# tombultreys/ptv_interpolation

Measured on AMD Instinct MI355X. Metric: Mvoxels/s interpolated + achieved HBM GB/s, 512³ grid / 5M particles IDW, higher is better.
Workload: dtype f64

## Files before the change

### include/ptv_api.h

```cpp
#ifndef PTV_API_H
#define PTV_API_H

#include <stdint.h>

#ifdef __cplusplus
extern "C" {
#endif

#define PTV_API_VERSION 11

#define PTV_OK 0
#define PTV_E_ARG -1
#define PTV_E_HIP -2
#define PTV_E_NOMEM -3
#define PTV_E_UNSUPPORTED -4
#define PTV_E_INEXACT -5
#define PTV_E_SINGULAR -6

#define PTV_METHOD_IDW 0
#define PTV_METHOD_SIBSON 1
#define PTV_METHOD_NEAREST 2
#define PTV_METHOD_IDW_RADIUS 3

#define PTV_RBF_LINEAR 0
// ... 238 lines not shown
typedef struct {
    int64_t n_fluid, n_dirichlet;
    int32_t itn;
    int32_t info;
    int32_t solver;
    int32_t anchor_plane;
    double bnorm, rnorm;
    double sum_abs_fx, sum_abs_fy, sum_abs_fz, sum_w;
    double ms_force, ms_divergence, ms_solve;
    double ms_iter_median;
    double ms_total;
} ptv_pressure_stats;

int ptv_version(void);
int ptv_abi_sizes(int64_t out6[6]);
int ptv_abi_sizes2(int64_t out3[3]);
int ptv_abi_sizes3(int64_t out1[1]);
int ptv_abi_sizes4(int64_t out2[2]);
int ptv_abi_sizes5(int64_t out2[2]);
int ptv_abi_sizes6(int64_t out2[2]);
int ptv_abi_sizes7(int64_t out2[2]);
int ptv_abi_sizes8(int64_t out4[4]);
int ptv_abi_sizes9(int64_t out2[2]);
const char *ptv_last_error(void);
int ptv_device_count(int *out);
int ptv_init(int device, ptv_ctx **out);
int ptv_free(ptv_ctx *ctx);

int ptv_interp_knn(ptv_ctx *ctx, const ptv_particles *p, const ptv_grid *g,
                   const ptv_knn_params *prm, double *U, double *V, double *W,
                   ptv_stats *st);

int ptv_interp_knn_dev(ptv_ctx *ctx, const ptv_particles *p, const ptv_grid *g,
                       const ptv_knn_params *prm, double *U, double *V, double *W,
                       void *stream, ptv_stats *st);

int ptv_interp_rbf_local(ptv_ctx *ctx, const ptv_particles *p, const ptv_grid *g,
                         const ptv_rbf_params *prm, double *U, double *V, double *W,
                         ptv_stats *st);

int ptv_interp_rbf_local_dev(ptv_ctx *ctx, const ptv_particles *p, const ptv_grid *g,
                             const ptv_rbf_params *prm, double *U, double *V, double *W,
                             void *stream, ptv_stats *st);

int ptv_interp_linear(ptv_ctx *ctx, const ptv_particles *p, const ptv_grid *g,
                      const ptv_linear_params *prm, double *U, double *V, double *W,
// ... 97 lines not shown
                         const double *Fz, double *D);

int ptv_force_divergence_dev(ptv_ctx *ctx, const ptv_pressure_params *prm, const double *Fx, const double *Fy,
                             const double *Fz, double *D, void *stream);

int ptv_poisson_solve(ptv_ctx *ctx, const ptv_pressure_params *prm, const double *rhs, const double *Fx,
                      const double *Fy, const double *Fz, const uint8_t *dirichlet, double *X,
                      ptv_pressure_stats *st);

int ptv_poisson_solve_dev(ptv_ctx *ctx, const ptv_pressure_params *prm, const double *rhs, const double *Fx,
                          const double *Fy, const double *Fz, const uint8_t *dirichlet, double *X, void *stream,
                          ptv_pressure_stats *st);

int ptv_pressure_recover(ptv_ctx *ctx, const ptv_pressure_params *prm, const double *U, const double *V,
                         const double *W, double *P, ptv_pressure_stats *st);

int ptv_pressure_recover_dev(ptv_ctx *ctx, const ptv_pressure_params *prm, const double *U, const double *V,
                             const double *W, double *P, void *stream, ptv_pressure_stats *st);

int ptv_last_stats(ptv_ctx *ctx, ptv_stats *st);

int ptv_debug_stamps(ptv_ctx *ctx, int mode, double *out23);

#ifdef __cplusplus
}
#endif

#endif
```

### ptv_interpolation_amd/_lib.py

```python
from __future__ import annotations

import ctypes as C
import os
import threading

import numpy as np

HERE = os.path.dirname(os.path.abspath(__file__))
_DEFAULT_LIB = os.path.join(HERE, "libptv_amd.so")
LIB_PATH = os.environ.get("PTV_LIB", _DEFAULT_LIB)

PTV_OK = 0
PTV_E_ARG = -1
PTV_E_HIP = -2
PTV_E_NOMEM = -3
PTV_E_UNSUPPORTED = -4
PTV_E_INEXACT = -5
PTV_E_SINGULAR = -6

METHOD_IDW = 0
METHOD_SIBSON = 1
METHOD_NEAREST = 2
METHOD_IDW_RADIUS = 3

# ... 282 lines not shown
    "ptv_interface_drag": (C.c_int, [C.c_void_p, C.POINTER(DragParams)] + [C.c_void_p] * 6 + [_dp]),
    "ptv_interface_drag_dev": (C.c_int, [C.c_void_p, C.POINTER(DragParams)] + [C.c_void_p] * 7 + [_dp]),
    "ptv_gradient_sums": (C.c_int, [C.c_void_p, C.POINTER(FlowParams), C.c_void_p, _dp]),
    "ptv_gradient_sums_dev": (C.c_int, [C.c_void_p, C.POINTER(FlowParams), C.c_void_p, C.c_void_p, _dp]),
    "ptv_abi_sizes8": (C.c_int, [C.POINTER(C.c_int64)]),
    "ptv_edt": (C.c_int, [C.c_void_p, C.POINTER(EdtParams)] + [C.c_void_p] * 3 + [C.POINTER(EdtStats)]),
    "ptv_edt_dev": (C.c_int, [C.c_void_p, C.POINTER(EdtParams)] + [C.c_void_p] * 4 + [C.POINTER(EdtStats)]),
    "ptv_align_score": (C.c_int, [C.c_void_p, C.POINTER(AlignParams)] + [C.c_void_p] * 4 + [_dp]),
    "ptv_align_score_dev": (C.c_int, [C.c_void_p, C.POINTER(AlignParams)] + [C.c_void_p] * 5 + [_dp]),
    "ptv_abi_sizes9": (C.c_int, [C.POINTER(C.c_int64)]),
    "ptv_force_field": (C.c_int, [C.c_void_p, C.POINTER(PressureParams)] + [_dp] * 6 + [C.POINTER(PressureStats)]),
    "ptv_force_field_dev": (C.c_int, [C.c_void_p, C.POINTER(PressureParams)] + [_dp] * 6 +
                            [C.c_void_p, C.POINTER(PressureStats)]),
    "ptv_force_divergence": (C.c_int, [C.c_void_p, C.POINTER(PressureParams)] + [_dp] * 4),
    "ptv_force_divergence_dev": (C.c_int, [C.c_void_p, C.POINTER(PressureParams)] + [_dp] * 4 + [C.c_void_p]),
    "ptv_poisson_solve": (C.c_int, [C.c_void_p, C.POINTER(PressureParams)] + [_dp] * 4 + [_u8p, _dp,
                                                                                           C.POINTER(PressureStats)]),
    "ptv_poisson_solve_dev": (C.c_int, [C.c_void_p, C.POINTER(PressureParams)] + [_dp] * 4 +
                              [_u8p, _dp, C.c_void_p, C.POINTER(PressureStats)]),
    "ptv_pressure_recover": (C.c_int, [C.c_void_p, C.POINTER(PressureParams)] + [_dp] * 4 +
                             [C.POINTER(PressureStats)]),
    "ptv_pressure_recover_dev": (C.c_int, [C.c_void_p, C.POINTER(PressureParams)] + [_dp] * 4 +
                                 [C.c_void_p, C.POINTER(PressureStats)]),
    "ptv_last_stats": (C.c_int, [C.c_void_p, C.POINTER(Stats)]),
    "ptv_debug_stamps": (C.c_int, [C.c_void_p, C.c_int, C.POINTER(C.c_double)]),
}

_lib = None
_lock = threading.Lock()


class PtvError(RuntimeError):
    def __init__(self, code, msg):
        super().__init__(f"ptv error {code}: {msg}")
        self.code = code
        self.msg = msg


def lib():
    global _lib
    with _lock:
        if _lib is None:
            if not os.path.exists(LIB_PATH):
                raise ImportError(
                    f"{LIB_PATH} not found: build it with `python -m ptv_interpolation_amd.build` "
                    "(hipcc, gfx950). The k-NN path has no CPU fallback.")
# ... 74 lines not shown
    out = (C.c_int64 * 2)()
    check(lib().ptv_abi_sizes6(out))
    return list(out), [C.sizeof(FlowParams), C.sizeof(FlowStats)]


def abi_sizes7():
    out = (C.c_int64 * 2)()
    check(lib().ptv_abi_sizes7(out))
    return list(out), [C.sizeof(DragParams), C.sizeof(DragStats)]


def abi_sizes8():
    out = (C.c_int64 * 4)()
    check(lib().ptv_abi_sizes8(out))
    return list(out), [C.sizeof(EdtParams), C.sizeof(EdtStats), C.sizeof(AlignParams), C.sizeof(AlignRecord)]


def abi_sizes9():
    out = (C.c_int64 * 2)()
    check(lib().ptv_abi_sizes9(out))
    return list(out), [C.sizeof(PressureParams), C.sizeof(PressureStats)]


def edt_check_shape(shape):
    if len(shape) != 3:
        raise NotImplementedError(f"the GPU distance transform is 3-D only (got {len(shape)}-D)")
    if sum(int(n) * int(n) for n in shape) >= 2**31:
        raise NotImplementedError(f"shape {tuple(shape)}: nz^2 + ny^2 + nx^2 must be below 2^31 "
                                  "(squared distances are 32-bit on the GPU)")
    return tuple(int(n) for n in shape)


def drag_label_table(labels):
    lab = np.asarray(labels)
    if lab.ndim != 1 or lab.size == 0:
        raise ValueError("labels must be a non-empty 1-D sequence")
    if lab.dtype.kind not in "biu":
        raise NotImplementedError(f"labels of dtype {lab.dtype} (GPU path: integers or bool)")
    lab = lab.astype(np.int64) if lab.dtype != np.uint64 else lab
    if lab.max() > np.iinfo(np.int32).max or lab.min() < np.iinfo(np.int32).min:
        raise NotImplementedError("labels outside the int32 range are not supported on the GPU path")
    if lab.min() <= 0:
        raise NotImplementedError("labels must be positive on the GPU path (0 is the fluid)")
    table, slot = np.unique(lab.astype(np.int32), return_inverse=True)
    return np.ascontiguousarray(table), slot.reshape(-1)

# ... 107 lines not shown
        check(L.ptv_init(int(device), C.byref(h)))
        self.h = h
        self.device = int(device)

    @classmethod
    def get(cls, device: int = 0) -> "Context":
        with _lock:
            ctx = cls._cache.get(device)
        if ctx is None:
            ctx = cls(device)
            with _lock:
                cls._cache[device] = ctx
        return ctx

    def close(self):
        if self.h:
            lib().ptv_free(self.h)
            self.h = None

    def last_stats(self) -> dict:
        st = Stats()
        check(lib().ptv_last_stats(self.h, C.byref(st)))
        return st.as_dict()

    def debug_stamps(self, mode=2):
        out = (C.c_double * 23)()
        check(lib().ptv_debug_stamps(self.h, int(mode), out))
        keys = ("setup", "seeds", "rows", "copy", "compute", "epilogue", "candidates", "merges", "rounds",
                "passes", "kept")
        v = list(out)
        return {"waves": v[0], "mean": dict(zip(keys, v[1:12])), "max": dict(zip(keys, v[12:23]))}

    def sample_mask(self, raw, raw_axes, axes=None, grid_points=None, shape=None, z_range=None):
        rw = np.ascontiguousarray(raw, dtype=np.uint8)
        rnz, rny, rnx = rw.shape
        rax, ray, raz = (np.ascontiguousarray(a, dtype=np.float64).ravel() for a in raw_axes)
        M = MaskGrid(rnx, rny, rnz, rw.ctypes.data_as(_u8p), as_dp(rax), as_dp(ray), as_dp(raz))
        keep = [rw, rax, ray, raz]
        if axes is not None:
            ax, ay, az = (np.ascontiguousarray(a, dtype=np.float64).ravel() for a in axes)
            nx, ny, nz = len(ax), len(ay), len(az)
            keep += [ax, ay, az]
            G = Grid(nx, ny, nz, as_dp(ax), as_dp(ay), as_dp(az), None, None, None, 0, nz)
        else:
            nz, ny, nx = shape
            gp = [np.ascontiguousarray(a, dtype=np.float64).ravel() for a in grid_points]
# ... 626 lines not shown
```

### ptv_interpolation_amd/build.py

```python
from __future__ import annotations

import os
import shutil
import subprocess
import sys
from concurrent.futures import ThreadPoolExecutor

HERE = os.path.dirname(os.path.abspath(__file__))
CSRC = os.path.join(HERE, "csrc")
INCLUDE = os.path.join(os.path.dirname(HERE), "include")
LIB = os.path.join(HERE, "libptv_amd.so")
BUILD = os.path.join(HERE, "csrc", "_build")
KNN_PARTS = ["ptv_knn_k" + g + ".hip" for g in "abcdefgh"]
SOURCES = (["ptv_api.cpp", "ptv_search.cpp", "ptv_run_knn.cpp", "ptv_run_chunked.cpp", "ptv_bin.hip", "ptv_knn.hip"] + KNN_PARTS +
           ["ptv_rbf.hip"] + ["ptv_rbf_ns_" + g + ".hip" for g in "abcd"] +
           ["ptv_div.hip", "ptv_flow.hip", "ptv_drag.hip", "ptv_edt.hip", "ptv_clean.hip", "ptv_variational.hip", "ptv_pressure.hip", "ptv_mask.hip", "ptv_filter.hip", "ptv_linear.hip", "ptv_knn_big.hip"])
ARCH = os.environ.get("PTV_OFFLOAD_ARCH", "gfx950")
EXTRA = {f: ["-mllvm", "-pragma-unroll-threshold=1000000"] for f in ["ptv_rbf.hip"] + ["ptv_rbf_ns_" + g + ".hip" for g in "abcd"]}
for _f in ["ptv_rbf.hip"] + ["ptv_rbf_ns_" + g + ".hip" for g in "abcd"]:
    EXTRA[_f] += ["-mllvm", "-disable-machine-licm"]

COMMON = ["-O3", "-fPIC", "-std=c++17", "-ffp-contract=off", f"--offload-arch={ARCH}",
          "-I", INCLUDE, "-I", CSRC, "-Wno-unused-result"]
EXTRA_FLAGS = os.environ.get("PTV_EXTRA_FLAGS", "").split()
TAG = os.environ.get("PTV_BUILD_TAG", "")
if TAG:
    LIB = os.path.join(os.path.dirname(HERE), "ab", f"libptv_{TAG}.so")
    BUILD = os.path.join(HERE, "csrc", "_build_" + TAG)
    EXTRA_FLAGS.append("-DPTV_DEV_KNOBS=1")


def hipcc() -> str:
    for cand in (os.environ.get("HIPCC"), shutil.which("hipcc"), "/opt/rocm/bin/hipcc"):
        if cand and os.path.exists(cand):
            return cand
    raise RuntimeError("hipcc not found (ROCm toolchain required to build libptv_amd.so)")

# ... 44 lines not shown
```

### ptv_interpolation_amd/csrc/ptv_api.cpp

```cpp
#include <cstdio>
#include <hip/hip_runtime.h>

#include <algorithm>
#include <cmath>
#include <memory>
#include <string>
#include <thread>

#include <sys/mman.h>
#include <vector>

#include "ptv_ctx.hpp"

namespace ptv {

static thread_local std::string g_last_error;
void set_error(const std::string &msg) { g_last_error = msg; }

}

using namespace ptv;

extern "C" {

// ... 72 lines not shown
    out2[1] = (int64_t)sizeof(ptv_drag_stats);
    return PTV_OK;
}

int ptv_abi_sizes8(int64_t out4[4]) {
    if (!out4) {
        set_error("ptv_abi_sizes8: out is NULL");
        return PTV_E_ARG;
    }
    out4[0] = (int64_t)sizeof(ptv_edt_params);
    out4[1] = (int64_t)sizeof(ptv_edt_stats);
    out4[2] = (int64_t)sizeof(ptv_align_params);
    out4[3] = (int64_t)sizeof(ptv_align_record);
    return PTV_OK;
}

int ptv_abi_sizes9(int64_t out2[2]) {
    if (!out2) {
        set_error("ptv_abi_sizes9: out is NULL");
        return PTV_E_ARG;
    }
    out2[0] = (int64_t)sizeof(ptv_pressure_params);
    out2[1] = (int64_t)sizeof(ptv_pressure_stats);
    return PTV_OK;
}

const char *ptv_last_error(void) { return g_last_error.c_str(); }

int ptv_device_count(int *out) {
    if (!out) {
        set_error("ptv_device_count: out is NULL");
        return PTV_E_ARG;
    }
    int n = 0;
    hipError_t e = hipGetDeviceCount(&n);
    if (e != hipSuccess) n = 0;
    *out = n;
    return PTV_OK;
}

int ptv_init(int device, ptv_ctx **out) {
    if (!out) {
        set_error("ptv_init: out is NULL");
        return PTV_E_ARG;
    }
    *out = nullptr;
// ... 501 lines not shown
            if (r[0] == 0 && r[2] == 0 && r[5] == 0) continue;
            ++nrec;
            double v[nv];
            for (int f = 0; f < 6; ++f) v[f] = (double)r[f];
            v[6] = (double)(r[6] & 0xffffffffULL);
            v[7] = (double)(r[6] >> 32);
            v[8] = (double)(r[7] & 0xffffULL);
            v[9] = (double)((r[7] >> 16) & 0xffffULL);
            v[10] = (double)(r[7] >> 32);
            for (int f = 0; f < nv; ++f) {
                sum[f] += v[f];
                mx[f] = std::max(mx[f], v[f]);
            }
        }
        out[0] = (double)nrec;
        for (int f = 0; f < nv; ++f) {
            out[1 + f] = nrec ? sum[f] / (double)nrec : 0.0;
            out[1 + nv + f] = mx[f];
        }
    }
    return PTV_OK;
}

int ptv_divergence_dev(ptv_ctx *c, const ptv_div_params *prm, const void *U, const void *V, const void *W,
                       void *out, void *stream, ptv_stats *st) {
    DivArgs a{};
    PTV_TRY(div_args(c, prm, U, V, W, out, a));
    hipStream_t s = stream ? (hipStream_t)stream : c->stream;
    PTV_TRY(run_div(c, a, U, V, W, prm->fluid_mask, out, s));
    c->last.n_voxels = (prm->z_end - prm->z_begin) * prm->nx * prm->ny;
    if (st) *st = c->last;
    return PTV_OK;
}

int ptv_divergence(ptv_ctx *c, const ptv_div_params *prm, const void *U, const void *V, const void *W, void *out,
                   ptv_stats *st) {
    DivArgs a{};
    PTV_TRY(div_args(c, prm, U, V, W, out, a));
    hipStream_t s = c->stream;
    Event ev[4];
    const size_t ts = a.field_f32 ? 4 : 8, rs = a.result_f32 ? 4 : 8;
    const int64_t nfull = prm->nz * prm->nx * prm->ny;
    const int64_t nout = (prm->z_end - prm->z_begin) * prm->nx * prm->ny;
    PTV_TRY(ev[0].record(s));
    const void *src[3] = {U, V, W};
    for (int i = 0; i < 3; ++i) {
// ... 1352 lines not shown
```

### ptv_interpolation_amd/csrc/ptv_ctx.hpp

```cpp
#pragma once

#include <vector>

#include "../../include/ptv_api.h"
#include "ptv_clean.hpp"
#include "ptv_kernels.hpp"
#include "ptv_knn_big.hpp"
#include "ptv_own.hpp"
#include "ptv_pressure.hpp"
#include "ptv_variational.hpp"

namespace ptv {

constexpr int kMaxLattice = 6;

struct CullCache {
    std::vector<double> key;
    std::vector<double> key_host;
    DevBuf<double> key_dev;
    bool kept_valid = false;
    int64_t kept = 0;
    double bbox[6] = {0, 0, 0, 0, 0, 0};
};

}

struct ptv_ctx {
    int device = 0;
    ptv::Stream stream;
    ptv::Event ev_knn0, ev_knn1, ev_bin0, ev_bin1, ev_lat1;
    ptv::Event ev_main0, ev_cull0, ev_cull1;
    bool cull_timed = false;
    bool timed_pending = false;
    ptv::BigScratch big;
    ptv::DevBuf<double> pin[6], axes, qpts[3], out[3];
    ptv::DevBuf<double> rbf_huge;
    ptv::DevBuf<uint8_t> mask;
    ptv::DevBuf<uint32_t> code, perm, count, start, scanp;
    ptv::DevBuf<uint32_t> bin_keys;
    ptv::DevBuf<uint8_t> bin_temp;
    ptv::DevBuf<double4> prec, pval;
    ptv::DevBuf<double> bbox_part, bbox_out;
    ptv::DevBuf<unsigned long long> dbg;
    ptv::DevBuf<double> lat_axes[ptv::kMaxLattice], lat_dk[ptv::kMaxLattice];
    ptv::DevBuf<float4> lat_recs[ptv::kMaxLattice];
    ptv::DevBuf<int> lat_order[ptv::kMaxLattice];
    ptv::DevBuf<double> lat_okeys;
    ptv::DevBuf<uint32_t> lat_split;
    ptv::DevBuf<double> cmap[2], cdk, ccols, cfp;
    ptv::DevBuf<unsigned long long> ckeys;
    ptv::CullMap cmap_geo{};
    int cdk_n[3] = {0, 0, 0};
    bool cmap_valid = false;
    ptv::CullCache ccache;
    ptv::DevBuf<uint32_t> slots;
    ptv::DevBuf<int> rbf_pw, rbf_status;
    ptv::DevBuf<uint32_t> rbf_nslist;
    ptv::DevBuf<int> rbf_cflag;
    ptv::DevBuf<double> smooth;
    ptv::DevBuf<uint8_t> fld[4];
    ptv::DevBuf<double> mask_axes;
    ptv::DevBuf<int> mask_tabs;
    ptv::DevBuf<uint8_t> mask_raw, mask_out;
    ptv::DevBuf<uint8_t> bnd_ping, bnd_pong;
    ptv::DevBuf<unsigned long long> bnd_counts;
    ptv::DevBuf<double> bnd_xyz;
    ptv::DevBuf<uint8_t> flt_keep;
    ptv::DevBuf<uint32_t> flt_code, flt_perm, flt_count, flt_start, flt_scanp;
    ptv::DevBuf<double> flt_kth, flt_spd;
    ptv::DevBuf<double> cull[6], cull_win;
// ... 119 lines not shown
```

### ptv_interpolation_amd/csrc/ptv_kernels.hpp

```cpp
#pragma once

#include "../../include/ptv_api.h"
#include "ptv_common.hpp"

namespace ptv {

int launch_bbox(const double *const px[3], int64_t n, const double *const qa[3], const int64_t qn[3],
                double *d_partials, int max_blocks, double *d_out6, hipStream_t s,
                const uint32_t *d_n = nullptr);

struct BinSortScratch {
    uint32_t *keys = nullptr;
    void *temp = nullptr;
    size_t temp_bytes = 0;
};
size_t bin_sort_temp_bytes(int64_t n, size_t m);
int launch_bin(const CellGrid &cg, const double *const px[3], const double *const pv[3], int64_t n,
               uint32_t *d_code, uint32_t *d_perm, uint32_t *d_count, uint32_t *d_start,
               uint32_t *d_scan_partials, double4 *d_prec, double4 *d_pval, hipStream_t s,
               const BinSortScratch *ss = nullptr);

size_t scan_partials_needed(size_t m);

size_t cull_blocks(int64_t n);
// ... 51 lines not shown
    int method;
    int k;
    double power, eps;
    uint32_t flags;
    double r0;
    int mode = kModeInterp;
    CoarseBound cb;
    float4 *kd_recs = nullptr;
    int lz0 = -1;
    uint32_t *slots = nullptr;
    double radius = 0.0;
    FilterEpilogue fe;
    const int *order = nullptr;
    unsigned int *rep_cnt = nullptr;
    uint32_t *rep_list = nullptr;
    int rep_cap = 0;
    unsigned int *h_rep = nullptr;
    int64_t *n_repair = nullptr;
    const unsigned long long *gate = nullptr;
    double gate_halo = 0.0;
    int split = 0;
    int split_blocks = 0;
    uint32_t *split_out = nullptr;
};

inline size_t kdist_split_slots(int split, int split_blocks, int kmax) {
    return (size_t)split_blocks * 4 * (size_t)split * (size_t)kmax * 64;
}

int launch_block_order(const double *dk_coarse, const int nc[3], int nx, int ny, int nz, double unit, int *order,
                       double *keys, hipStream_t s);

int launch_count_bound(const CellGrid &g, const uint32_t *cstart, const double *ax, const double *ay,
                       const double *az, int nx, int ny, int nz, int k, double r0, double *out, hipStream_t s);

int launch_subsample(const double *in, int n, int step, double *out, int nout, hipStream_t s);
constexpr int kMaxSubsampleLevels = 8;
struct SubsampleBatch {
    const double *base[3];
    int n0[3];
    int nlev;
    int n[kMaxSubsampleLevels][3];
    double *out[kMaxSubsampleLevels][3];
};
int launch_subsample_levels(const SubsampleBatch &b, int step, hipStream_t s);
int launch_concat3(const double *a, int na, const double *b, int nb, const double *c, int nc, double *out,
                   hipStream_t s);

int launch_halo_need(const double *lax, const double *lay, const double *laz, int nx, int ny, int nz,
                     const double *dk, const double *win, double mg, unsigned long long *out, hipStream_t s);

int kmax_for(int k);
extern unsigned long long *g_dbg;
extern long long g_dbg_cap;

int launch_knn(const KnnLaunch &a, const Binned &b, const double *ax, const double *ay, const double *az,
               const double *qx, const double *qy, const double *qz, const uint8_t *mask, double *U, double *V,
               double *W, hipStream_t s);

struct DivArgs {
    int nx, ny, nz;
    int z_begin, z_end;
    int edge_lo, edge_hi;
    int field_f32;
    int result_f32;
    double dx, dy, dz;
    int ntx = 0, nty = 0, ntiles = 0;
    int xcd = 0;
};

int launch_divergence(const DivArgs &a, const void *U, const void *V, const void *W, const uint8_t *M, void *out,
                      hipStream_t s);

constexpr int kFlowRows = 16;
struct FlowArgs {
    int nx, ny, nz;
    int z_begin, z_end;
// ... 163 lines not shown
```

### ptv_interpolation_amd/csrc/ptv_knn.hip

```cpp
#include "ptv_knn_impl.hpp"

namespace ptv {

unsigned long long *g_dbg = nullptr;
long long g_dbg_cap = 0;

__device__ __forceinline__ int count_inside(const CellGrid &g, const uint32_t *__restrict__ cstart, double qx,
                                            double qy, double qz, double R, int lane) {
    const double Ri = R - g.mg;
    if (Ri <= 0.0) return 0;
    const double R2 = Ri * Ri;
    const int ry0 = clampi(floor((qy - Ri - g.o[1]) * g.ic[1]), g.nc[1]);
    const int ry1 = clampi(floor((qy + Ri - g.o[1]) * g.ic[1]), g.nc[1]);
    const int rz0 = clampi(floor((qz - Ri - g.o[2]) * g.ic[2]), g.nc[2]);
    const int rz1 = clampi(floor((qz + Ri - g.o[2]) * g.ic[2]), g.nc[2]);
    const int nyr = ry1 - ry0 + 1;
    const int nrows = nyr * (rz1 - rz0 + 1);
    int cnt = 0;
    for (int row = lane; row < nrows; row += 64) {
        const int ccy = ry0 + row % nyr, ccz = rz0 + row / nyr;
        const double y0 = g.o[1] + (double)ccy * g.cs[1], y1 = g.o[1] + (double)(ccy + 1) * g.cs[1];
        const double z0 = g.o[2] + (double)ccz * g.cs[2], z1 = g.o[2] + (double)(ccz + 1) * g.cs[2];
        const double fy = fmax(fabs(y0 - qy), fabs(y1 - qy)), fz = fmax(fabs(z0 - qz), fabs(z1 - qz));
        const double h2 = fy * fy + fz * fz;
// ... 343 lines not shown
        diag2 += e * e;
    }
    ka.rall = sqrt(diag2) * (1.0 + 1e-9) + a.cg.mg;
    const long long nblocks = (long long)ka.ntxb * ka.nty * ka.ntz;
    if (nblocks > 0x7fffffffLL || (keys && nblocks >= (1LL << 30))) {
        set_error("grid too large for one launch");
        return PTV_E_ARG;
    }
    ka.nblocks = (int)nblocks;
    int B = 1;
    while (B < 31 && (1LL << B) < b.n) ++B;
    ka.smask = (uint32_t)((1ULL << B) - 1ULL);
    ka.kscale = 1.0 + std::ldexp(1.0, B - 51);
    ka.rep_cnt = nullptr;
    ka.rep_list = nullptr;
    ka.rep_cap = 0;
    ka.tiles = nullptr;
    ka.ntiles = 0;
    ka.split = 0;
    ka.split_tiles = 0;
    ka.split_out = nullptr;
    ka.split_lb = 0;
    ka.order_skip = 0;
    if (a.mode == kModeKDist && a.split > 1 && a.split_blocks > 0 && a.order != nullptr && a.split_out != nullptr) {
        const int nsb = (int)std::min<long long>(a.split_blocks, nblocks);
        KnnKernelArgs ks = ka;
        ks.split = a.split;
        ks.split_tiles = nsb * 4;
        ks.split_out = a.split_out;
        PTV_HIP(hipMemsetAsync(a.split_out, 0xff, kdist_split_slots(a.split, nsb, km) * sizeof(uint32_t), s));
        const long long sblocks = ((long long)ks.split_tiles * a.split + 3) / 4;
        const long long total = sblocks + (nblocks - nsb);
        if (total > 0x7fffffffLL) {
            set_error("split lattice launch too large");
            return PTV_E_ARG;
        }
        ks.nblocks = (int)total;
        ks.split_lb = (int)sblocks;
        ks.order_skip = (int)(nsb - sblocks);
        int rc = launch_kmax(km, false, grid_for(total), s, ks, b, ax, ay, az, qx, qy, qz, mask, U, V, W);
        if (rc != PTV_OK) return rc;
        ks.mode = kModeKDistMerge;
        return launch_kmax(km, false, grid_for(nsb), s, ks, b, ax, ay, az, qx, qy, qz, mask, U, V, W);
    }
    const bool repair = keys && a.mode != kModeKDist && a.mode != kModeRadius;
    if (repair) {
// ... 30 lines not shown
```

### ptv_interpolation_amd/csrc/ptv_knn_impl.hpp

```cpp
#pragma once
#include <hip/hip_runtime.h>

#include <cfloat>
#include <cstdlib>
#include <algorithm>
#include <cmath>
#include <utility>

#include "../../include/ptv_api.h"
#include "ptv_kernels.hpp"
#include "ptv_median.hpp"
#include "ptv_wave.hpp"

namespace ptv {

#ifndef PTV_SUBBALL_RUNS
#define PTV_SUBBALL_RUNS 1
#endif
#ifndef PTV_KNN_WAVES
#define PTV_KNN_WAVES 4
#endif
#ifndef PTV_KNN_WAVES_BIG
#define PTV_KNN_WAVES_BIG 2
#endif
// ... 81 lines not shown
    CoarseBound cb;
    float4 *kd_recs;
    int lz0;
    uint32_t *slots;
    int seed_n;
    int nblocks;
    double radius;
    FilterEpilogue fe;
    const int *order;
    uint32_t smask;
    double kscale;
    unsigned int *rep_cnt;
    uint32_t *rep_list;
    int rep_cap;
    const uint32_t *tiles;
    int ntiles;
    const unsigned long long *gate;
    double gate_halo;
    int split;
    int split_tiles;
    uint32_t *split_out;
    int split_lb;
    int order_skip;
};

__device__ __forceinline__ double make_key(bool has, double e2, uint32_t slot, uint32_t smask) {
    const unsigned long long bits = (unsigned long long)__double_as_longlong(e2);
    uint32_t lo = ((uint32_t)bits & ~smask) | slot;
    uint32_t hi = (uint32_t)(bits >> 32);
    lo = has ? lo : 0u;
    hi = has ? hi : 0x7ff00000u;
    return __longlong_as_double((long long)(((unsigned long long)hi << 32) | lo));
}

__device__ __forceinline__ uint32_t key_slot(double key, uint32_t smask) {
    return (uint32_t)__double_as_longlong(key) & smask;
}

__device__ __forceinline__ bool same_trunc(double a, double b, uint32_t smask) {
    const unsigned long long x = (unsigned long long)(__double_as_longlong(a) ^ __double_as_longlong(b));
    return (x & ~(unsigned long long)smask) == 0ull;
}

template <int KMAX>
__device__ __forceinline__ void insert_key(double (&bd)[KMAX], double key) {
    double cd = key;
// ... 1832 lines not shown
```

### ptv_interpolation_amd/csrc/ptv_search.cpp

```cpp
#include <algorithm>
#include <cmath>
#include <cstdio>
#include <cstdlib>
#include <cstring>
#include <vector>

#include "ptv_ctx.hpp"

namespace ptv {

namespace {

constexpr double kDefaultOccupancySmallK = 16.0;
constexpr double kDefaultXRefSmallK = 12.0;
constexpr double kDefaultOccupancy = 1.2;
constexpr double kDefaultOccupancyLargeK = 8.0;
constexpr double kDefaultXRefLargeK = 4.0;
constexpr double kDefaultR0Scale = 1.0;
constexpr long long kMaxCells = 1LL << 28;
constexpr long long kLatticeStopPoints = 50000;
constexpr size_t kSeedBytesMax = 40ULL << 30;
constexpr int kLatticeSplit = 16;
constexpr long long kLatticeSplitMinBlocks = 64;
constexpr long long kLatticeSplitDiv = 128;
// ... 220 lines not shown
            if (!lattice_level_above(nl) && !(exact_finest && nlat == 1 && nmin >= 2)) break;
            Lat &L = lat[nlat];
            for (int d = 0; d < 3; ++d) L.n[d] = n[d] <= 1 ? 1 : (n[d] - 1 + kLatticeStep - 1) / kLatticeStep + 1;
            PTV_TRY(c->lat_axes[nlat].ensure((size_t)L.n[0] + L.n[1] + L.n[2]));
            PTV_TRY(c->lat_dk[nlat].ensure((size_t)L.n[0] * L.n[1] * L.n[2]));
            L.ax = c->lat_axes[nlat].p;
            L.ay = L.ax + L.n[0];
            L.az = L.ay + L.n[1];
            L.dk = c->lat_dk[nlat].p;
            L.recs = nullptr;
            double *dst[3] = {L.ax, L.ay, L.az};
            for (int d = 0; d < 3; ++d) {
                sb.n[nlat][d] = L.n[d];
                sb.out[nlat][d] = dst[d];
                n[d] = L.n[d];
            }
            ++nlat;
        }
        sb.nlev = nlat;
        if (nlat > 0) PTV_TRY(launch_subsample_levels(sb, kLatticeStep, s));
    }

    const KnnLaunch kl = search_launch(g, prm, pr);
    PTV_TRY(c->ev_knn0.record(s));
    for (int l = nlat - 1; l >= 0; --l) {
        if (l == nlat - 1) {
            PTV_TRY(launch_count_bound(pr.cg, c->start.p, lat[l].ax, lat[l].ay, lat[l].az, lat[l].n[0], lat[l].n[1],
                                       lat[l].n[2], prm->k, pr.r0, lat[l].dk, s));
            continue;
        }
        const size_t nrec = (size_t)lat[l].n[0] * lat[l].n[1] * lat[l].n[2] * prm->k;
        if ((l > 0 || main_seeds) && nrec * sizeof(float4) <= kSeedBytesMax) {
            PTV_TRY(c->lat_recs[l].ensure(nrec));
            lat[l].recs = c->lat_recs[l].p;
        }
        KnnLaunch ll = kl;
        const char *no_order = dev_knob("PTV_NO_LAT_ORDER");
        if (!(no_order && no_order[0] == '1')) {
            const long long nb = (long long)(((lat[l].n[0] + 3) / 4 + 3) / 4) * ((lat[l].n[1] + 3) / 4) *
                                 ((lat[l].n[2] + 3) / 4);
            PTV_TRY(c->lat_order[l].ensure((size_t)nb));
            PTV_TRY(c->lat_okeys.ensure((size_t)nb + 1));
            PTV_TRY(launch_block_order(lat[l + 1].dk, lat[l + 1].n, lat[l].n[0], lat[l].n[1], lat[l].n[2], pr.r0,
                                       c->lat_order[l].p, c->lat_okeys.p, s));
            ll.order = c->lat_order[l].p;
            if (const char *e = dev_knob("PTV_DBG_ORDER"))
                if (l == 0)
                    PTV_TRY(dump_lattice(e, lat[1].n, lat[1].dk, (size_t)lat[1].n[0] * lat[1].n[1] * lat[1].n[2],
                                         ll.order, (size_t)nb, s));
            int split = kLatticeSplit;
            long long sblk = std::min<long long>(nb, std::max<long long>(kLatticeSplitMinBlocks, nb / kLatticeSplitDiv));
            if (const char *e = dev_knob("PTV_LAT_SPLIT")) split = std::atoi(e);
            if (const char *e = dev_knob("PTV_LAT_SPLIT_BLOCKS")) sblk = std::min<long long>(nb, std::atoll(e));
            if (split > 1)
                sblk = std::min<long long>(sblk, (long long)(kLatticeSplitBytesMax / sizeof(uint32_t) /
                                                             kdist_split_slots(split, 1, kmax_for(prm->k))));
            if (split > 1 && sblk > 0) {
                PTV_TRY(c->lat_split.ensure(kdist_split_slots(split, (int)sblk, kmax_for(prm->k))));
                ll.split = split;
                ll.split_blocks = (int)sblk;
                ll.split_out = c->lat_split.p;
            }
        }
        ll.kd_recs = lat[l].recs;
        ll.nx = lat[l].n[0];
        ll.ny = lat[l].n[1];
        ll.nz = lat[l].n[2];
        ll.z0 = 0;
        ll.z1 = lat[l].n[2];
        ll.mode = kModeKDist;
        ll.flags = 0;
        ll.cb = bound_of(lat[l + 1]);
        if (const char *e = dev_knob("PTV_LAT_SEEDS"))
            if (e[0] == '0') ll.cb.recs = nullptr;
        PTV_TRY(launch_knn(ll, pr.b, lat[l].ax, lat[l].ay, lat[l].az, nullptr, nullptr, nullptr, nullptr, lat[l].dk,
                           lat[l].dk, lat[l].dk, s));
    }
    pr.cb = nlat > 0 ? bound_of(lat[0]) : CoarseBound{};
    PTV_TRY(c->ev_lat1.record(s));
    if (const char *e = dev_knob("PTV_DBG_LATDK"))
        if (nlat > 0)
            PTV_TRY(dump_lattice(e, lat[0].n, lat[0].dk, (size_t)lat[0].n[0] * lat[0].n[1] * lat[0].n[2], nullptr, 0, s));
    return PTV_OK;
}

int fill_launch(ptv_ctx *c, const ptv_grid *g, const SearchParams *prm, hipStream_t s, const Prepared &pr,
                KnnLaunch &kl) {
    kl = search_launch(g, prm, pr);
    kl.cb = pr.cb;
    PTV_TRY(c->ev_main0.record(s));
    const int64_t nz = g->z_end - g->z_begin;
    ptv_stats &ls = c->last;
    ls = ptv_stats{};
    ls.n_particles = pr.b.n;
    ls.n_voxels = nz * g->nx * g->ny;
    ls.n_cells = (int64_t)pr.cg.nc[0] * pr.cg.nc[1] * pr.cg.nc[2];
    for (int a = 0; a < 3; ++a) {
        ls.cells[a] = pr.cg.nc[a];
        ls.cell_size[a] = pr.cg.cs[a];
    }
    ls.r0 = pr.r0;
// ... 88 lines not shown
```

Before: 8580.

## Add per-point lattice k-distance kernel with wave-cooperative fallback for wide searches

Adds a new kernel that computes lattice k-distances per point. Each lane walks its own candidate cell rows with radius doubling, bounded by the coarser lattice's k-distance and its seed records. Points whose search spans too many rows are deferred and then processed one at a time by the whole wave, and a counter records how many were deferred. The lattice split path is turned off when this kernel is active. A debug API that exports the lattice level and binned particles is also added.

```diff
diff --git a/include/ptv_api.h b/include/ptv_api.h
--- a/include/ptv_api.h
+++ b/include/ptv_api.h
@@ -284,6 +284,7 @@
 int ptv_abi_sizes7(int64_t out2[2]);
 int ptv_abi_sizes8(int64_t out4[4]);
 int ptv_abi_sizes9(int64_t out2[2]);
+int ptv_abi_sizes10(int64_t out2[2]);
 const char *ptv_last_error(void);
 int ptv_device_count(int *out);
 int ptv_init(int device, ptv_ctx **out);
@@ -427,6 +428,10 @@
 
 int ptv_debug_stamps(ptv_ctx *ctx, int mode, double *out23);
 
+#define PTV_LATTICE_INFO_WORDS 9
+int ptv_debug_lattice(ptv_ctx *ctx, int64_t *info, double *dk, int64_t dk_cap, float *recs, int64_t recs_cap,
+                      double *binned, int64_t binned_cap);
+
 #ifdef __cplusplus
 }
 #endif
diff --git a/ptv_interpolation_amd/_lib.py b/ptv_interpolation_amd/_lib.py
--- a/ptv_interpolation_amd/_lib.py
+++ b/ptv_interpolation_amd/_lib.py
@@ -328,6 +328,9 @@
                              [C.POINTER(PressureStats)]),
     "ptv_pressure_recover_dev": (C.c_int, [C.c_void_p, C.POINTER(PressureParams)] + [_dp] * 4 +
                                  [C.c_void_p, C.POINTER(PressureStats)]),
+    "ptv_abi_sizes10": (C.c_int, [C.POINTER(C.c_int64)]),
+    "ptv_debug_lattice": (C.c_int, [C.c_void_p, C.POINTER(C.c_int64), _dp, C.c_int64, C.c_void_p, C.c_int64, _dp,
+                          C.c_int64]),
     "ptv_last_stats": (C.c_int, [C.c_void_p, C.POINTER(Stats)]),
     "ptv_debug_stamps": (C.c_int, [C.c_void_p, C.c_int, C.POINTER(C.c_double)]),
 }
@@ -448,6 +451,15 @@
     return list(out), [C.sizeof(PressureParams), C.sizeof(PressureStats)]
 
 
+LATTICE_INFO_WORDS = 9
+
+
+def abi_sizes10():
+    out = (C.c_int64 * 2)()
+    check(lib().ptv_abi_sizes10(out))
+    return list(out), [LATTICE_INFO_WORDS, 16]
+
+
 def edt_check_shape(shape):
     if len(shape) != 3:
         raise NotImplementedError(f"the GPU distance transform is 3-D only (got {len(shape)}-D)")
@@ -601,6 +613,28 @@
         st = Stats()
         check(lib().ptv_last_stats(self.h, C.byref(st)))
         return st.as_dict()
+
+    def debug_lattice(self, records=True):
+        info = (C.c_int64 * LATTICE_INFO_WORDS)()
+        check(lib().ptv_debug_lattice(self.h, info, None, 0, None, 0, None, 0))
+        nx, ny, nz, k, has_recs, searched, points, coop, nb = (int(v) for v in info)
+        res = {"shape": (nz, ny, nx), "k": k, "searched": bool(searched), "points": bool(points),
+               "coop_points": coop, "dk": None, "offsets": None, "slots": None, "binned": None}
+        n = nx * ny * nz
+        if n == 0:
+            return res
+        dk = np.empty(n, dtype=np.float64)
+        rec = np.empty((n * k, 4), dtype=np.float32) if (records and has_recs) else None
+        binned = np.empty((nb, 4), dtype=np.float64)
+        check(lib().ptv_debug_lattice(self.h, info, dk.ctypes.data_as(_dp), n,
+                                      rec.ctypes.data if rec is not None else None, n * k if rec is not None else 0,
+                                      binned.ctypes.data_as(_dp), nb))
+        res["dk"] = dk.reshape(nz, ny, nx)
+        res["binned"] = binned
+        if rec is not None:
+            res["offsets"] = rec[:, :3].reshape(nz, ny, nx, k, 3).copy()
+            res["slots"] = rec[:, 3].copy().view(np.uint32).reshape(nz, ny, nx, k)
+        return res
 
     def debug_stamps(self, mode=2):
         out = (C.c_double * 23)()
diff --git a/ptv_interpolation_amd/build.py b/ptv_interpolation_amd/build.py
--- a/ptv_interpolation_amd/build.py
+++ b/ptv_interpolation_amd/build.py
@@ -12,7 +12,7 @@
 LIB = os.path.join(HERE, "libptv_amd.so")
 BUILD = os.path.join(HERE, "csrc", "_build")
 KNN_PARTS = ["ptv_knn_k" + g + ".hip" for g in "abcdefgh"]
-SOURCES = (["ptv_api.cpp", "ptv_search.cpp", "ptv_run_knn.cpp", "ptv_run_chunked.cpp", "ptv_bin.hip", "ptv_knn.hip"] + KNN_PARTS +
+SOURCES = (["ptv_api.cpp", "ptv_search.cpp", "ptv_run_knn.cpp", "ptv_run_chunked.cpp", "ptv_bin.hip", "ptv_knn.hip", "ptv_lattice.hip"] + KNN_PARTS +
            ["ptv_rbf.hip"] + ["ptv_rbf_ns_" + g + ".hip" for g in "abcd"] +
            ["ptv_div.hip", "ptv_flow.hip", "ptv_drag.hip", "ptv_edt.hip", "ptv_clean.hip", "ptv_variational.hip", "ptv_pressure.hip", "ptv_mask.hip", "ptv_filter.hip", "ptv_linear.hip", "ptv_knn_big.hip"])
 ARCH = os.environ.get("PTV_OFFLOAD_ARCH", "gfx950")
diff --git a/ptv_interpolation_amd/csrc/ptv_api.cpp b/ptv_interpolation_amd/csrc/ptv_api.cpp
--- a/ptv_interpolation_amd/csrc/ptv_api.cpp
+++ b/ptv_interpolation_amd/csrc/ptv_api.cpp
@@ -118,6 +118,16 @@
     }
     out2[0] = (int64_t)sizeof(ptv_pressure_params);
     out2[1] = (int64_t)sizeof(ptv_pressure_stats);
+    return PTV_OK;
+}
+
+int ptv_abi_sizes10(int64_t out2[2]) {
+    if (!out2) {
+        set_error("ptv_abi_sizes10: out is NULL");
+        return PTV_E_ARG;
+    }
+    out2[0] = (int64_t)PTV_LATTICE_INFO_WORDS;
+    out2[1] = (int64_t)sizeof(float4);
     return PTV_OK;
 }
 
@@ -665,6 +675,51 @@
     return PTV_OK;
 }
 
+int ptv_debug_lattice(ptv_ctx *c, int64_t *info, double *dk, int64_t dk_cap, float *recs, int64_t recs_cap,
+                      double *binned, int64_t binned_cap) {
+    if (!c || !info) {
+        set_error("ptv_debug_lattice: NULL context or info");
+        return PTV_E_ARG;
+    }
+    PTV_HIP(hipSetDevice(c->device));
+    PTV_HIP(hipStreamSynchronize(c->stream));
+    const ptv::LatticeInfo &li = c->lat_info;
+    const int64_t np = (int64_t)li.n[0] * li.n[1] * li.n[2];
+    unsigned int coop = 0;
+    if (li.points && c->lat_coop.p) PTV_HIP(hipMemcpy(&coop, c->lat_coop.p, sizeof(coop), hipMemcpyDeviceToHost));
+    info[0] = li.n[0];
+    info[1] = li.n[1];
+    info[2] = li.n[2];
+    info[3] = li.k;
+    info[4] = li.recs != nullptr;
+    info[5] = li.searched;
+    info[6] = li.points;
+    info[7] = (int64_t)coop;
+    info[8] = li.n_binned;
+    if (dk) {
+        if (!li.dk || dk_cap < np) {
+            set_error("ptv_debug_lattice: no lattice level, or dk holds fewer than its points");
+            return PTV_E_ARG;
+        }
+        PTV_HIP(hipMemcpy(dk, li.dk, (size_t)np * sizeof(double), hipMemcpyDeviceToHost));
+    }
+    if (recs) {
+        if (!li.recs || recs_cap < np * li.k) {
+            set_error("ptv_debug_lattice: no seed records, or recs holds fewer than points * k records");
+            return PTV_E_ARG;
+        }
+        PTV_HIP(hipMemcpy(recs, li.recs, (size_t)np * li.k * sizeof(float4), hipMemcpyDeviceToHost));
+    }
+    if (binned) {
+        if (!li.prec || binned_cap < li.n_binned) {
+            set_error("ptv_debug_lattice: no binned particles, or binned holds fewer than their count");
+            return PTV_E_ARG;
+        }
+        PTV_HIP(hipMemcpy(binned, li.prec, (size_t)li.n_binned * sizeof(double4), hipMemcpyDeviceToHost));
+    }
+    return PTV_OK;
+}
+
 int ptv_divergence_dev(ptv_ctx *c, const ptv_div_params *prm, const void *U, const void *V, const void *W,
                        void *out, void *stream, ptv_stats *st) {
     DivArgs a{};
diff --git a/ptv_interpolation_amd/csrc/ptv_ctx.hpp b/ptv_interpolation_amd/csrc/ptv_ctx.hpp
--- a/ptv_interpolation_amd/csrc/ptv_ctx.hpp
+++ b/ptv_interpolation_amd/csrc/ptv_ctx.hpp
@@ -21,6 +21,17 @@
     bool kept_valid = false;
     int64_t kept = 0;
     double bbox[6] = {0, 0, 0, 0, 0, 0};
+};
+
+struct LatticeInfo {
+    int n[3] = {0, 0, 0};
+    int k = 0;
+    const double *dk = nullptr;
+    const float4 *recs = nullptr;
+    bool searched = false;
+    bool points = false;
+    const double4 *prec = nullptr;
+    int64_t n_binned = 0;
 };
 
 }
@@ -46,6 +57,8 @@
     ptv::DevBuf<float4> lat_recs[ptv::kMaxLattice];
     ptv::DevBuf<int> lat_order[ptv::kMaxLattice];
     ptv::DevBuf<double> lat_okeys;
+    ptv::DevBuf<unsigned int> lat_coop;
+    ptv::LatticeInfo lat_info;
     ptv::DevBuf<uint32_t> lat_split;
     ptv::DevBuf<double> cmap[2], cdk, ccols, cfp;
     ptv::DevBuf<unsigned long long> ckeys;
diff --git a/ptv_interpolation_amd/csrc/ptv_kernels.hpp b/ptv_interpolation_amd/csrc/ptv_kernels.hpp
--- a/ptv_interpolation_amd/csrc/ptv_kernels.hpp
+++ b/ptv_interpolation_amd/csrc/ptv_kernels.hpp
@@ -97,6 +97,8 @@
     int split = 0;
     int split_blocks = 0;
     uint32_t *split_out = nullptr;
+    bool points = false;
+    unsigned int *lat_coop = nullptr;
 };
 
 inline size_t kdist_split_slots(int split, int split_blocks, int kmax) {
@@ -128,6 +130,10 @@
 int kmax_for(int k);
 extern unsigned long long *g_dbg;
 extern long long g_dbg_cap;
+
+struct KnnKernelArgs;
+int launch_lattice_points(int km, dim3 grid, hipStream_t s, const KnnKernelArgs &ka, const Binned &b,
+                          const double *ax, const double *ay, const double *az, double *U);
 
 int launch_knn(const KnnLaunch &a, const Binned &b, const double *ax, const double *ay, const double *az,
                const double *qx, const double *qy, const double *qz, const uint8_t *mask, double *U, double *V,
diff --git a/ptv_interpolation_amd/csrc/ptv_knn.hip b/ptv_interpolation_amd/csrc/ptv_knn.hip
--- a/ptv_interpolation_amd/csrc/ptv_knn.hip
+++ b/ptv_interpolation_amd/csrc/ptv_knn.hip
@@ -389,6 +389,14 @@
     ka.split_out = nullptr;
     ka.split_lb = 0;
     ka.order_skip = 0;
+    ka.lat_coop = a.lat_coop;
+    if (a.points) {
+        if (a.mode != kModeKDist || keys || !a.separable || mask != nullptr) {
+            set_error("the per-point lattice kernel serves separable k-distance launches with k <= 12");
+            return PTV_E_ARG;
+        }
+        return launch_lattice_points(km, grid_for(nblocks), s, ka, b, ax, ay, az, U);
+    }
     if (a.mode == kModeKDist && a.split > 1 && a.split_blocks > 0 && a.order != nullptr && a.split_out != nullptr) {
         const int nsb = (int)std::min<long long>(a.split_blocks, nblocks);
         KnnKernelArgs ks = ka;
diff --git a/ptv_interpolation_amd/csrc/ptv_knn_impl.hpp b/ptv_interpolation_amd/csrc/ptv_knn_impl.hpp
--- a/ptv_interpolation_amd/csrc/ptv_knn_impl.hpp
+++ b/ptv_interpolation_amd/csrc/ptv_knn_impl.hpp
@@ -127,6 +127,7 @@
     uint32_t *split_out;
     int split_lb;
     int order_skip;
+    unsigned int *lat_coop;
 };
 
 __device__ __forceinline__ double make_key(bool has, double e2, uint32_t slot, uint32_t smask) {
diff --git a/ptv_interpolation_amd/csrc/ptv_lattice.hip b/ptv_interpolation_amd/csrc/ptv_lattice.hip
--- /dev/null
+++ b/ptv_interpolation_amd/csrc/ptv_lattice.hip
@@ -0,0 +1,282 @@
+#include "ptv_knn_impl.hpp"
+#include "ptv_lattice_index.hpp"
+
+namespace ptv {
+
+namespace {
+
+constexpr int kLatMaxPass = 64;
+
+__device__ __forceinline__ double bcast(double v, int src) {
+    const long long b = __double_as_longlong(v);
+    const int lo = __builtin_amdgcn_readlane((int)(b & 0xffffffffLL), src);
+    const int hi = __builtin_amdgcn_readlane((int)(b >> 32), src);
+    return __longlong_as_double(((long long)hi << 32) | (unsigned int)lo);
+}
+
+__device__ __forceinline__ double sqrt_up_cells(double x, double ic, double cs) {
+    return (double)sqrtf_up((float)(x * ic * ic * (1.0 + 2.384185791015625e-07))) * cs * (1.0 + 1e-7);
+}
+
+template <int KMAX>
+__device__ __forceinline__ void walk_row(const CellGrid &g, const double4 *__restrict__ prec,
+                                         const uint32_t *__restrict__ cstart, int cy, int cz, double qx, double qy,
+                                         double qz, double ub2, double (&bd)[KMAX], int (&bp)[KMAX]) {
+    double thr = dmin(bd[KMAX - 1], ub2);
+    const double rw = sqrt_up_cells(thr, g.ic[1], g.cs[1]) + 2.0 * g.mg;
+    const double gy = axis_gap(cy, g.o[1], g.cs[1], qy, qy), gz = axis_gap(cz, g.o[2], g.cs[2], qz, qz);
+    const double g2 = gy * gy + gz * gz, rw2 = rw * rw;
+    if (g2 > rw2) return;
+    const double h = sqrt_up_cells(rw2 - g2, g.ic[1], g.cs[1]) + g.mg;
+    int cx0, cx1;
+    lat_span(qx, h, g.o[0], g.ic[0], g.nc[0], cx0, cx1);
+    if (cx0 > cx1) return;
+    const size_t row = ((size_t)cz * g.nc[1] + cy) * g.nc[0];
+    const uint32_t p0 = cstart[row + cx0], p1 = cstart[row + cx1 + 1];
+    for (uint32_t p = p0; p < p1; ++p) {
+        const double4 c = prec[p];
+        const double dx = qx - c.x, dy = qy - c.y, dz = qz - c.z;
+        const double e2 = (dx * dx + dy * dy) + dz * dz;
+        if (e2 < thr) {
+            insert<KMAX>(bd, bp, e2, (int)p);
+            thr = dmin(bd[KMAX - 1], ub2);
+        }
+    }
+}
+
+}
+
+template <int KMAX>
+__global__ __launch_bounds__(256) void k_lattice_points(KnnKernelArgs a, const double4 *__restrict__ prec,
+                                                        const uint32_t *__restrict__ cstart,
+                                                        const double *__restrict__ ax, const double *__restrict__ ay,
+                                                        const double *__restrict__ az, double *__restrict__ U) {
+    __shared__ uint32_t lds_tab[4][1024];
+    __shared__ float lds_sx[4][64], lds_sy[4][64], lds_sz[4][64];
+    const int lane = threadIdx.x & 63;
+    const int wid = threadIdx.x >> 6;
+    const int lb = (int)(blockIdx.y * gridDim.x + blockIdx.x);
+    if (lb >= a.nblocks) return;
+    int b = a.order != nullptr ? a.order[lb] : xcd_block(lb, a.nblocks);
+    b = __builtin_amdgcn_readfirstlane(b);
+    const int bx = b % a.ntxb, rr = b / a.ntxb;
+    const int ty = rr % a.nty, tz = rr / a.nty;
+    const int tx = __builtin_amdgcn_readfirstlane(bx * 4 + wid);
+    if (tx >= a.ntx) return;
+    const int ix = tx * 4 + (lane & 3), iy = ty * 4 + ((lane >> 2) & 3), iz = a.z0 + tz * 4 + (lane >> 4);
+    const bool valid = ix < a.nx && iy < a.ny && iz < a.z1;
+    const int cx = min(ix, a.nx - 1), cy = min(iy, a.ny - 1), cz = min(iz, a.z1 - 1);
+    const size_t vo = ((size_t)(cz - a.z0) * a.ny + cy) * a.nx + cx;
+    const double qx = ax[cx], qy = ay[cy], qz = az[cz];
+    const CellGrid &g = a.cg;
+
+    const int j0x = __builtin_amdgcn_readfirstlane(cx >> kLatticeShift);
+    const int j0y = __builtin_amdgcn_readfirstlane(cy >> kLatticeShift);
+    const int j0z = __builtin_amdgcn_readfirstlane((cz - a.lz0) >> kLatticeShift);
+    auto lattice_ub = [&]() -> double {
+        double u = INFINITY;
+        if (a.cb.dk == nullptr) return u;
+#pragma unroll
+        for (int c = 0; c < 8; ++c) {
+            const int jx = min(j0x + (c & 1), a.cb.n[0] - 1);
+            const int jy = min(j0y + ((c >> 1) & 1), a.cb.n[1] - 1);
+            const int jz = min(j0z + (c >> 2), a.cb.n[2] - 1);
+            const double ex = qx - a.cb.ax[jx], ey = qy - a.cb.ay[jy], ez = qz - a.cb.az[jz];
+            const double e = sqrt((ex * ex + ey * ey) + ez * ez) * (1.0 + 1e-12);
+            const double D = a.cb.dk[((size_t)jz * a.cb.n[1] + jy) * a.cb.n[0] + jx];
+            u = fmin(u, D + e);
+        }
+        return u * (1.0 + 1e-9) + g.mg;
+    };
+
+    double ub = INFINITY, ub2 = INFINITY;
+    if (a.cb.recs != nullptr) {
+        const int cc = lane >> 3, j = lane & 7;
+        const int jx = min(j0x + (cc & 1), a.cb.n[0] - 1);
+        const int jy = min(j0y + ((cc >> 1) & 1), a.cb.n[1] - 1);
+        const int jz = min(j0z + (cc >> 2), a.cb.n[2] - 1);
+        float4 seed = make_float4(0.f, 0.f, 0.f, __uint_as_float(0xffffffffu));
+        if (j < min(a.k, 8)) seed = a.cb.recs[(((size_t)jz * a.cb.n[1] + jy) * a.cb.n[0] + jx) * a.k + j];
+        const double scx = a.cb.ax[jx], scy = a.cb.ay[jy], scz = a.cb.az[jz];
+        auto ext = [](const double *axv, int i0, int imax, double &lo, double &hi) {
+            const double v0 = axv[i0], v1 = axv[min(i0 + 1, imax)], v2 = axv[min(i0 + 2, imax)],
+                         v3 = axv[min(i0 + 3, imax)];
+            lo = uniform(fmin(fmin(v0, v1), fmin(v2, v3)));
+            hi = uniform(fmax(fmax(v0, v1), fmax(v2, v3)));
+        };
+        double bx0, bx1, by0, by1, bz0, bz1;
+        ext(ax, tx * 4, a.nx - 1, bx0, bx1);
+        ext(ay, ty * 4, a.ny - 1, by0, by1);
+        ext(az, a.z0 + tz * 4, a.z1 - 1, bz0, bz1);
+        const double tcx = 0.5 * (bx0 + bx1), tcy = 0.5 * (by0 + by1), tcz = 0.5 * (bz0 + bz1);
+        const float qfx = (float)(qx - tcx), qfy = (float)(qy - tcy), qfz = (float)(qz - tcz);
+        const double bhalf =
+            0.5 * sqrt_up(((bx1 - bx0) * (bx1 - bx0) + (by1 - by0) * (by1 - by0)) + (bz1 - bz0) * (bz1 - bz0));
+        uint32_t *tab = lds_tab[wid];
+        float *sx = lds_sx[wid], *sy = lds_sy[wid], *sz = lds_sz[wid];
+        const uint32_t sl = __float_as_uint(seed.w);
+        const bool has = sl != 0xffffffffu;
+        const uint32_t hsh = (sl * 2654435761u) >> 22;
+        if (has) tab[hsh] = (uint32_t)lane;
+        wave_lds_sync();
+        const bool uniq = has && tab[hsh] == (uint32_t)lane;
+        const unsigned long long um = __builtin_amdgcn_ballot_w64(uniq);
+        const int nu = __builtin_popcountll(um);
+        const int pos = __builtin_amdgcn_mbcnt_hi((unsigned)(um >> 32), __builtin_amdgcn_mbcnt_lo((unsigned)um, 0u));
+        double pm = 0.0;
+        if (uniq) {
+            const float ex = seed.x + (float)(scx - tcx), ey = seed.y + (float)(scy - tcy), ez = seed.z + (float)(scz - tcz);
+            sx[pos] = ex;
+            sy[pos] = ey;
+            sz[pos] = ez;
+            pm = ((double)fabsf(ex) + (double)fabsf(ey) + (double)fabsf(ez)) * (1.0 + 1e-6);
+        }
+        const double Ms = uniform(wave_max(pm)) + bhalf;
+        wave_lds_sync();
+        float sd[KMAX];
+#pragma unroll
+        for (int q = 0; q < KMAX; ++q) sd[q] = INFINITY;
+        for (int i = 0; i < nu; ++i) {
+            const float ex = qfx - sx[i], ey = qfy - sy[i], ez = qfz - sz[i];
+            const float s2 = __fmaf_rn(ez, ez, __fmaf_rn(ey, ey, ex * ex));
+#pragma unroll
+            for (int q = KMAX - 1; q > 0; --q) sd[q] = __builtin_amdgcn_fmed3f(sd[q - 1], sd[q], s2);
+            sd[0] = fminf(sd[0], s2);
+        }
+        float kth = sd[0];
+#pragma unroll
+        for (int q = 1; q < KMAX; ++q)
+            if (q == a.k - 1) kth = sd[q];
+        if (kth < INFINITY && kth >= 1e-30f) {
+            const double dl = Ms * 1.9073486328125e-06;
+            const double st2 = ((double)kth * (1.0 + 9.5367431640625e-07) + (2.0 * Ms * dl + dl * dl)) * (1.0 + 1e-12);
+            ub2 = st2;
+            ub = sqrt(st2) * (1.0 + 1e-12);
+        }
+    }
+    if (!(ub < INFINITY)) {
+        ub = lattice_ub();
+        ub2 = ub * ub;
+    }
+    if (!(ub < a.rall) || !(ub2 < INFINITY)) {
+        ub = a.rall;
+        ub2 = a.rall * a.rall;
+    }
+
+    double bd[KMAX];
+    int bp[KMAX];
+    double R = fmin(a.r0, ub);
+    if (!(R > 0.0)) R = ub;
+    int ly = 0, hy = -1, lz = 0, hz = -1;
+    bool deferred = false;
+    if (valid) {
+        for (int pass = 0; pass < kLatMaxPass; ++pass) {
+            const bool fin = !(R < ub) || pass == kLatMaxPass - 1;
+            const double lim2 = fin ? ub2 : R * R;
+            const double rb = (fin ? ub : R) * (1.0 + 1e-7) + 2.0 * g.mg;
+            lat_span(qy, rb, g.o[1], g.ic[1], g.nc[1], ly, hy);
+            lat_span(qz, rb, g.o[2], g.ic[2], g.nc[2], lz, hz);
+            if (lat_deferred(hy - ly + 1, hz - lz + 1)) {
+                deferred = true;
+                break;
+            }
+#pragma unroll
+            for (int j = 0; j < KMAX; ++j) {
+                bd[j] = j < a.kpad ? -1.0 : INFINITY;
+                bp[j] = -1;
+            }
+            for (int z = lz; z <= hz; ++z)
+                for (int y = ly; y <= hy; ++y) walk_row<KMAX>(g, prec, cstart, y, z, qx, qy, qz, lim2, bd, bp);
+            if (fin || bd[KMAX - 1] < INFINITY) break;
+            R *= 2.0;
+        }
+        if (!deferred) kdist_out<KMAX, false>(a, prec, bd, bp, qx, qy, qz, vo, U);
+    }
+
+    unsigned long long dm = __builtin_amdgcn_ballot_w64(deferred);
+    if (dm == 0) return;
+    if (a.lat_coop != nullptr && lane == 0) atomicAdd(a.lat_coop, (unsigned int)__builtin_popcountll(dm));
+    while (dm != 0) {
+        const int t = __builtin_ctzll(dm);
+        dm &= dm - 1;
+        const double tqx = bcast(qx, t), tqy = bcast(qy, t), tqz = bcast(qz, t);
+        const double tub = bcast(ub, t), tub2 = bcast(ub2, t);
+        double tR = bcast(R, t);
+        const unsigned int tvo_lo = (unsigned int)__builtin_amdgcn_readlane((int)(vo & 0xffffffffu), t);
+        const unsigned int tvo_hi = (unsigned int)__builtin_amdgcn_readlane((int)(vo >> 32), t);
+        const size_t tvo = ((size_t)tvo_hi << 32) | tvo_lo;
+        for (int pass = 0; pass < kLatMaxPass; ++pass) {
+            const bool fin = !(tR < tub) || pass == kLatMaxPass - 1;
+            const double lim2 = fin ? tub2 : tR * tR;
+            const double rb = (fin ? tub : tR) * (1.0 + 1e-7) + 2.0 * g.mg;
+            int tly, thy, tlz, thz;
+            lat_span(tqy, rb, g.o[1], g.ic[1], g.nc[1], tly, thy);
+            lat_span(tqz, rb, g.o[2], g.ic[2], g.nc[2], tlz, thz);
+            const int tny = thy - tly + 1, tnz = thz - tlz + 1;
+#pragma unroll
+            for (int j = 0; j < KMAX; ++j) {
+                bd[j] = j < a.kpad ? -1.0 : INFINITY;
+                bp[j] = -1;
+            }
+            const int nrows = tny > 0 && tnz > 0 ? tny * tnz : 0;
+            for (int r = lane; r < nrows; r += 64)
+                walk_row<KMAX>(g, prec, cstart, tly + r % tny, tlz + r / tny, tqx, tqy, tqz, lim2, bd, bp);
+            int have = 0;
+#pragma unroll
+            for (int j = 0; j < KMAX; ++j) have += (bd[j] >= 0.0 && bd[j] < INFINITY) ? 1 : 0;
+            have = group_reduce<0x3f>(have, OpAdd{});
+            if (fin || have >= a.k) break;
+            tR *= 2.0;
+        }
+        double mp = -0.5;
+        int sp = 0x7fffffff;
+        float4 *o = a.kd_recs != nullptr ? a.kd_recs + tvo * (size_t)a.k : nullptr;
+        for (int it = 0; it < a.k; ++it) {
+            double cd = INFINITY;
+            int cs = 0x7fffffff;
+#pragma unroll
+            for (int j = KMAX - 1; j >= 0; --j) {
+                const bool gt = bd[j] < INFINITY && (bd[j] > mp || (bd[j] == mp && bp[j] > sp));
+                cd = gt ? bd[j] : cd;
+                cs = gt ? bp[j] : cs;
+            }
+            const double m = wave_min(cd);
+            const int smin = group_reduce<0x3f>(cd == m ? cs : 0x7fffffff, OpMin{});
+            const bool hasm = m < INFINITY;
+            if (o != nullptr) {
+                if (hasm && cd == m && cs == smin) {
+                    const double4 c = prec[cs];
+                    o[it] = make_float4((float)(c.x - tqx), (float)(c.y - tqy), (float)(c.z - tqz),
+                                        __uint_as_float((uint32_t)cs));
+                } else if (!hasm && lane == 0) {
+                    o[it] = make_float4(0.f, 0.f, 0.f, __uint_as_float(0xffffffffu));
+                }
+            }
+            if (it == a.k - 1 && lane == 0) U[tvo] = sqrt(m);
+            mp = m;
+            sp = hasm ? smin : 0x7fffffff;
+        }
+    }
+}
+
+int launch_lattice_points(int km, dim3 grid, hipStream_t s, const KnnKernelArgs &ka, const Binned &b,
+                          const double *ax, const double *ay, const double *az, double *U) {
+    switch (km) {
+#define PTV_CASE(K)                                                                                             \
+    case K:                                                                                                     \
+        hipLaunchKernelGGL((k_lattice_points<K>), grid, dim3(256), 0, s, ka, b.prec, b.cstart, ax, ay, az, U); \
+        break;
+        PTV_CASE(1)
+        PTV_CASE(4)
+        PTV_CASE(8)
+        PTV_CASE(12)
+#undef PTV_CASE
+        default:
+            set_error("no per-point lattice kernel for a list of length " + std::to_string(km));
+            return PTV_E_UNSUPPORTED;
+    }
+    PTV_HIP(hipGetLastError());
+    return PTV_OK;
+}
+
+}
diff --git a/ptv_interpolation_amd/csrc/ptv_lattice_index.hpp b/ptv_interpolation_amd/csrc/ptv_lattice_index.hpp
--- /dev/null
+++ b/ptv_interpolation_amd/csrc/ptv_lattice_index.hpp
@@ -0,0 +1,25 @@
+#pragma once
+
+#if defined(__HIPCC__)
+#define PTV_HD __host__ __device__
+#else
+#define PTV_HD
+#endif
+
+namespace ptv {
+
+#ifndef PTV_LAT_ROW_CAP
+#define PTV_LAT_ROW_CAP 48
+#endif
+constexpr int kLatRowCap = PTV_LAT_ROW_CAP;
+
+PTV_HD inline void lat_span(double q, double r, double o, double ic, int n, int &lo, int &hi) {
+    const double a = (q - r - o) * ic - 1.0, b = (q + r - o) * ic + 1.0;
+    const double top = (double)(n - 1);
+    lo = a >= 0.0 ? (a < top ? (int)a : n - 1) : 0;
+    hi = b < top ? (b >= 0.0 ? (int)b : 0) : n - 1;
+}
+
+PTV_HD inline bool lat_deferred(int ny, int nz) { return (long long)ny * (long long)nz > (long long)kLatRowCap; }
+
+}
diff --git a/ptv_interpolation_amd/csrc/ptv_search.cpp b/ptv_interpolation_amd/csrc/ptv_search.cpp
--- a/ptv_interpolation_amd/csrc/ptv_search.cpp
+++ b/ptv_interpolation_amd/csrc/ptv_search.cpp
@@ -266,6 +266,13 @@
     }
 
     const KnnLaunch kl = search_launch(g, prm, pr);
+    bool points = kmax_for(prm->k) <= 12 && prm->lattice_bounds == 2;
+    if (const char *e = dev_knob("PTV_LAT_POINTS")) points = kmax_for(prm->k) <= 12 && e[0] != '0';
+    c->lat_info = LatticeInfo{};
+    if (points && nlat > 1) {
+        PTV_TRY(c->lat_coop.ensure(1));
+        PTV_HIP(hipMemsetAsync(c->lat_coop.p, 0, sizeof(unsigned int), s));
+    }
     PTV_TRY(c->ev_knn0.record(s));
     for (int l = nlat - 1; l >= 0; --l) {
         if (l == nlat - 1) {
@@ -280,6 +287,8 @@
         }
         KnnLaunch ll = kl;
         const char *no_order = dev_knob("PTV_NO_LAT_ORDER");
+        ll.points = points;
+        ll.lat_coop = points ? c->lat_coop.p : nullptr;
         if (!(no_order && no_order[0] == '1')) {
             const long long nb = (long long)(((lat[l].n[0] + 3) / 4 + 3) / 4) * ((lat[l].n[1] + 3) / 4) *
                                  ((lat[l].n[2] + 3) / 4);
@@ -296,6 +305,7 @@
             long long sblk = std::min<long long>(nb, std::max<long long>(kLatticeSplitMinBlocks, nb / kLatticeSplitDiv));
             if (const char *e = dev_knob("PTV_LAT_SPLIT")) split = std::atoi(e);
             if (const char *e = dev_knob("PTV_LAT_SPLIT_BLOCKS")) sblk = std::min<long long>(nb, std::atoll(e));
+            if (points) split = 0;
             if (split > 1)
                 sblk = std::min<long long>(sblk, (long long)(kLatticeSplitBytesMax / sizeof(uint32_t) /
                                                              kdist_split_slots(split, 1, kmax_for(prm->k))));
@@ -321,6 +331,17 @@
                            lat[l].dk, lat[l].dk, s));
     }
     pr.cb = nlat > 0 ? bound_of(lat[0]) : CoarseBound{};
+    if (nlat > 0) {
+        LatticeInfo &li = c->lat_info;
+        for (int d = 0; d < 3; ++d) li.n[d] = lat[0].n[d];
+        li.k = prm->k;
+        li.dk = lat[0].dk;
+        li.recs = lat[0].recs;
+        li.searched = nlat > 1;
+        li.points = points && nlat > 1;
+        li.prec = pr.b.prec;
+        li.n_binned = pr.b.n;
+    }
     PTV_TRY(c->ev_lat1.record(s));
     if (const char *e = dev_knob("PTV_DBG_LATDK"))
         if (nlat > 0)
```

Measured after the change: 8481. -1.1%, worse.
